# opherlieber/rltime

Measured on AMD Instinct MI355X. Metric: sampled transitions/sec (= learner steps/sec x B x T), IQN-LSTM B=512 T=80 84x84x4, higher is better.
Workload: dtype f32

## Files before the change

### include/mirl.h

```cpp
#ifndef MIRL_H
#define MIRL_H

#include <stdint.h>

#ifdef __cplusplus
extern "C" {
#endif

#define MIRL_OK 0
#define MIRL_NEED_MORE 1
#define MIRL_ERR_ARG (-1)
#define MIRL_ERR_HIP (-2)
#define MIRL_ERR_STATE (-3)
#define MIRL_ERR_NOGPU (-4)

#define MIRL_MODE_UNIFORM 0
#define MIRL_MODE_PER 1

typedef struct mirl_replay mirl_replay;

typedef struct mirl_replay_config {
  int64_t size;
  int32_t num_envs;
  int32_t env_base;
// ... 128 lines not shown
                  double row_scale, float* row_loss, float* dq, float* td, void* stream);
int mirl_loss_iqn(int64_t M, int32_t N, int32_t Nt, int32_t A, const float* z,
                  const float* taus, const int64_t* actions, const float* targets,
                  const float* weights, double kappa, double row_scale,
                  float* row_loss, float* dz, float* abs_td, void* stream);

int mirl_q_target_c51(int64_t M, int32_t A, int32_t Z, const float* logits_target, const float* logits_select,
                      const float* support, const float* returns, const float* nsteps, const float* masks,
                      double gamma, double vmin, double vmax, double delta_z, int32_t projection,
                      float* targets, void* stream);
int mirl_loss_c51(int64_t M, int32_t A, int32_t Z, const float* logits, const int64_t* actions,
                  const float* targets, const float* weights, int32_t mode, double kappa, double row_scale,
                  float* row_loss, float* dlogits, float* report, void* stream);

int mirl_lstm_cell_fwd(int32_t B, int32_t H, float* gates, const float* c_in, const float* keep_next,
                       float* h_out, float* c_out, float* h_next, float* c_next, void* stream);
int mirl_lstm_seq_supported(int32_t T, int32_t B, int32_t H);
int mirl_lstm_seq_workspace_bytes(int32_t B, int32_t H, int64_t* bytes);
int mirl_lstm_seq_fwd(int32_t T, int32_t B, int32_t H, float* gx, const float* w_hh, const float* h0,
                      const float* c0, const float* keep, float* out, float* c_all, float* hm, float* cm,
                      float* h_last, float* c_last, int32_t save_gates, void* workspace, void* stream);
int mirl_lstm_seq_status(int32_t* status);
int mirl_lstm_seq_fwd_grid(int32_t B, int32_t H, int32_t* workgroups, int64_t* lds_bytes, int32_t* compute_units,
                           int32_t* per_compute_unit);
int mirl_lstm_seq_bwd_supported(int32_t T, int32_t B, int32_t H);
int mirl_lstm_seq_bwd_workspace_bytes(int32_t B, int32_t H, int64_t* bytes);
int mirl_lstm_seq_bwd(int32_t T, int32_t B, int32_t H, float* gates, const float* w_hh, const float* c_all,
                      const float* cm, const float* d_out, const float* keep, void* workspace, void* stream);
int mirl_lstm_cell_bwd(int32_t B, int32_t H, float* gates, const float* c_t, const float* c_in,
                       const float* d_out, const float* dh_rec, float* dc_rec, const float* keep_next,
                       int32_t first, void* stream);

int mirl_frames_to_f32_nhwc(int64_t N, int32_t C, int32_t HW, const uint8_t* src, float scale,
                            float* dst, void* stream);
int mirl_frames_to_f32_nhwc_ex(int64_t N, int32_t C, int32_t HW, const uint8_t* src, float scale,
                               float* dst, int32_t per_wg, int32_t flags, void* stream);

int mirl_conv1_u8_supported(int32_t C, int32_t H, int32_t W, int32_t F, int32_t K, int32_t S);
int mirl_conv1_u8_wpk_floats(int64_t* out);
int mirl_conv1_bf16_set(int32_t mode);
int mirl_conv1_wrw_bf16_set(int32_t mode);
int mirl_conv1_u8_fwd(int64_t N, int32_t H, int32_t W, const uint8_t* x, const float* weight,
                      int64_t ws_o, int64_t ws_c, int64_t ws_h, int64_t ws_w, const float* bias,
                      float scale, float* wpk, float* y, void* stream);
int mirl_conv1_u8_fwd_ex(int64_t N, int32_t H, int32_t W, const uint8_t* x, const float* weight,
                         int64_t ws_o, int64_t ws_c, int64_t ws_h, int64_t ws_w, const float* bias,
                         float scale, float* wpk, float* y, int32_t flags, void* stream);

int mirl_conv1_u8_wrw_scratch_floats(int64_t* out);
int mirl_conv1_u8_wrw(int64_t N, int32_t H, int32_t W, const uint8_t* x, const float* g, float scale,
                      float* scratch, float* dw, int64_t ws_o, int64_t ws_c, int64_t ws_h, int64_t ws_w,
                      void* stream);
int mirl_conv1_u8_wrw_ex(int64_t N, int32_t H, int32_t W, const uint8_t* x, const float* g, float scale,
                         float* scratch, float* dw, int64_t ws_o, int64_t ws_c, int64_t ws_h, int64_t ws_w,
                         int32_t flags, void* stream);
int mirl_conv1_u8_wrw_masked(int64_t N, int32_t H, int32_t W, const uint8_t* x, const float* dy, const float* y, float scale,
                             float* scratch, float* dw, int64_t ws_o, int64_t ws_c, int64_t ws_h, int64_t ws_w,
                             float* db, void* stream);

int mirl_conv2_bwd_data_supported(int32_t C, int32_t F, int32_t K, int32_t S, int32_t IH, int32_t IW,
                                  int32_t OH, int32_t OW);
int mirl_conv2_bwd_data(int64_t N, int32_t OH, int32_t OW, const float* g, const float* weight,
                        int64_t ws_o, int64_t ws_c, int64_t ws_h, int64_t ws_w, float* wpk, float* dx,
                        void* stream);
int mirl_conv2_bwd_data_wpk_floats(int64_t* floats);
int mirl_conv2_bwd_data_ex(int64_t N, int32_t OH, int32_t OW, const float* g, const float* weight, int64_t ws_o,
                           int64_t ws_c, int64_t ws_h, int64_t ws_w, float* wpk, int64_t wpk_floats, float* dx, int32_t pipe,
                           void* stream);
int mirl_conv3_bwd_data_supported(int32_t C, int32_t F, int32_t K, int32_t S, int32_t IH, int32_t IW, int32_t OH, int32_t OW);
int mirl_conv3_bwd_data_wpk_floats(int64_t* floats);
int mirl_conv3_bwd_data(int64_t N, int32_t OH, int32_t OW, const float* g, const float* weight, int64_t ws_o,
                        int64_t ws_c, int64_t ws_h, int64_t ws_w, float* wpk, int64_t wpk_floats, float* dx, void* stream);

int mirl_gemm3_supported(int32_t layout, int64_t M, int64_t N, int64_t K);
int mirl_gemm3_workspace_bytes(int32_t layout, int64_t M, int64_t N, int64_t K, int64_t* bytes);
int mirl_gemm3(int32_t layout, int64_t M, int64_t N, int64_t K, const float* A, int64_t lda,
               const float* B, int64_t ldb, float* C, int64_t ldc, const float* bias, int32_t relu,
               void* workspace, int64_t workspace_bytes, void* stream);
int mirl_gemm3_mid_set(int32_t mode);
int mirl_gemm3_nt_mul(int64_t M, int64_t N, int64_t K, const float* A, int64_t lda, const float* B,
                      int64_t ldb, float* C, int64_t ldc, const float* bias, int32_t relu,
                      const float* mul, int64_t ldmul, int32_t group_shift, float* pre, int64_t ldpre,
                      void* stream);
int mirl_gemm3_head_workspace_bytes(int64_t M, int64_t N, int64_t* bytes);
int mirl_gemm3_nt_head(int64_t M, int64_t N, int64_t K, const float* A, int64_t lda, const float* B, int64_t ldb,
                       float* C, int64_t ldc, const float* bias, int32_t relu, const float* w2, int32_t O,
                       const float* bias2, float* out2, int64_t ldo, void* workspace, int64_t workspace_bytes, void* stream);
int mirl_gemm3_nn_qp_partial_rows(int64_t M, int64_t* rows);
int mirl_gemm3_nn_qp(int64_t M, int64_t N, int64_t K, const float* A, int64_t lda, const float* B, int64_t ldb,
                     const float* emb, int64_t ldemb, const float* x, int64_t ldx, float* d_pre, int64_t ldd,
                     float* dx, int64_t lddx, float* db_partial, void* stream);

int mirl_conv3_fwd_supported(int32_t C, int32_t F, int32_t KH, int32_t KW, int32_t S, int32_t H, int32_t W);
int mirl_conv3_fwd(int64_t N, int32_t H, int32_t W, int32_t C, int32_t F, int32_t KH, int32_t KW, int32_t S,
                   const float* x, const float* w, const float* bias, int32_t relu, float* y, void* stream);

int mirl_conv_wrw_b3_supported(int32_t C, int32_t F, int32_t KH, int32_t KW, int32_t S, int32_t H, int32_t W);
int mirl_conv_wrw_b3_scratch_bytes(int32_t C, int32_t F, int32_t KH, int32_t KW, int64_t* bytes);
int mirl_conv_wrw_b3(int64_t N, int32_t H, int32_t W, int32_t C, int32_t F, int32_t KH, int32_t KW, int32_t S,
                     const float* x, const float* g, void* scratch, int64_t scratch_bytes, float* dw, void* stream);

int mirl_bias_relu_rows(int64_t rows, int32_t C, float* y, const float* bias, void* stream);
int mirl_colsum_blocks(int64_t rows, int32_t C, int32_t* blocks);
int mirl_relu_bwd_bias_rows(int64_t rows, int32_t C, const float* dy, const float* y, float* g,
                            float* db, float* partial, int32_t blocks, void* stream);
int mirl_cos_embed(int64_t rows, int32_t D, const float* tau, const float* freq, float* phi, void* stream);
int mirl_cos_embed_rng(int64_t rows, int32_t D, uint64_t seed, const uint64_t* step, const float* freq,
                       float* phi, float* tau_out, void* stream);
int mirl_iqn_mul_fwd(int64_t M, int32_t N, int32_t C, const float* x, const float* emb, float* out, void* stream);
int mirl_iqn_mul_bwd(int64_t M, int32_t N, int32_t C, const float* g, const float* emb, const float* x,
                     float* d_pre, float* dx, float* db, float* partial, int32_t blocks, void* stream);

int mirl_dueling_tail_bwd(int64_t M, int32_t H1, int32_t Hv, int32_t A, int32_t Q, const float* ga,
                          const float* gv, const float* wo, const float* wq, const float* both,
                          float* g, float* db, float* partial, int32_t blocks, void* stream);
int mirl_dueling_tail_bwd_w(int64_t M, int32_t H1, int32_t Hv, int32_t A, int32_t Q, const float* ga,
                            const float* gv, const float* wo, const float* wq, const float* both, float* g,
                            float* db, float* partial, int32_t blocks, float* dwj, float* partial_w,
                            void* stream);

int mirl_actor_head(int32_t E, int32_t N, int32_t A, const float* adv, const float* val, int32_t Q,
                    const double* eps, const double* expo, double eps_min, const float* u, const int64_t* rnd,
                    int32_t* actions, float* qvalues, float* eps_used, void* stream);
int mirl_actor_head_rng(int32_t E, int32_t N, int32_t A, const float* adv, int32_t adv_pitch, const float* val, int32_t Q,
                        const double* eps, const double* expo, double eps_min, uint64_t rng_seed,
                        const uint64_t* rng_step, int32_t* actions, float* qvalues, float* eps_used, void* stream);
int mirl_actor_head_c51(int32_t E, int32_t A, int32_t Z, const float* adv, int32_t adv_pitch, const float* val,
                        int32_t val_pitch, const float* support, const double* eps, const double* expo, double eps_min,
                        const float* u, const int64_t* rnd, uint64_t rng_seed, const uint64_t* rng_step,
                        int32_t* actions, float* qvalues, float* eps_used, void* stream);
int mirl_stack_shift(int32_t E, int32_t P, int32_t plane_bytes, const uint8_t* in, uint8_t* out,
                     const uint8_t* newest, const uint8_t* dones, void* stream);
#define MIRL_STEP_ADVANCE (~0ull)
int mirl_actor_pre(int32_t E, int32_t H, int32_t A, const float* rewards_raw, const uint8_t* dones,
                   const int32_t* actions, const float* h, const float* c, float* xh_tail, int64_t xh_pitch,
                   float* c_in, float* state_pack, float* initials, float* rewards_out, uint8_t* dones_out,
                   int32_t clip_rewards, float* ep_reward, int32_t* ep_len, float* out_reward, int32_t* out_len,
                   int32_t* action_counts, uint64_t* rng_step, uint64_t step, void* stream);
int mirl_synth_env_step(int32_t E, int64_t frame_bytes, const uint8_t* pool, int32_t pool_n, uint64_t* clock, int32_t slot,
                        uint64_t seed, float p_neg, float p_nonpos, float p_done, uint8_t* obs, float* rewards,
                        uint8_t* dones, void* stream);
int mirl_act_conv_supported(int32_t layer, int32_t Ci, int32_t Co, int32_t k, int32_t stride, int32_t Hi, int32_t Wi);
int mirl_act_conv_fwd(int32_t layer, int64_t frames, int32_t Hi, int32_t Wi, const float* x, const float* w_taps,
                      const float* bias, float* y, int64_t y_frame_pitch, void* stream);
int mirl_act_lstm_supported(int32_t E, int32_t H, int32_t K);
int mirl_act_lstm_workspace_bytes(int32_t E, int32_t H, int32_t K, int64_t* bytes);
int mirl_act_lstm_fwd(int32_t E, int32_t H, int32_t K, const float* xh, int64_t xh_pitch, const float* w, const float* bias,
                      const float* c_in, float* h_out, float* c_out, void* workspace, void* stream);
int mirl_act_embed(int32_t E, int32_t N, int32_t H, int32_t D, const float* h, const float* freq, const float* taus,
                   uint64_t seed, const uint64_t* step, const float* wq, const float* bq, float* x, float* tau_out, void* stream);
int mirl_act_head_supported(int32_t E, int32_t N, int32_t H, int32_t D, int32_t HID, int32_t NO);
int mirl_act_head_parts(int32_t HID, int32_t NO, int32_t* parts, int32_t* pitch);
int mirl_act_head_hidden(int32_t R, int32_t H, int32_t HID, int32_t NO, const float* x, const float* wfc, const float* bfc,
                         const float* wout, float* part, void* stream);
int mirl_act_head_select(int32_t E, int32_t N, int32_t A, int32_t parts, int32_t pitch, const float* part, const float* bout,
                         int32_t has_val, const double* eps, const double* expo, double eps_min, uint64_t rng_seed,
                         const uint64_t* rng_step, int32_t* actions, float* qvalues, void* stream);
int mirl_synth_env_step_pre(int32_t E, int64_t frame_bytes, const uint8_t* pool, int32_t pool_n, uint64_t* clock, int32_t slot,
                            uint64_t seed, float p_neg, float p_nonpos, float p_done, uint8_t* obs, float* rewards,
                            uint8_t* dones, int32_t H, int32_t A, const int32_t* actions, const float* h, const float* c,
                            float* xh_tail, int64_t xh_pitch, float* c_in, float* state_pack, float* initials,
                            float* rewards_out, uint8_t* dones_out, int32_t clip_rewards, float* ep_reward, int32_t* ep_len,
                            float* out_reward, int32_t* out_len, int32_t* action_counts, uint64_t* rng_step, uint64_t step,
                            void* stream);
int mirl_catch_env_step(int32_t E, int32_t P, int32_t S, int32_t G, int32_t V, int32_t A, const int32_t* actions, void* state,
                        uint64_t* clock, int32_t slot, uint64_t seed, int32_t reset_all, uint8_t* obs, float* rewards,
// ... 62 lines not shown
```

### rltime_amd/_lib.py

```python
import ctypes as C
import os

import torch

_HERE = os.path.dirname(os.path.abspath(__file__))
LIB_PATH = os.path.join(_HERE, "librltime_hip.so")

MIRL_OK = 0
MIRL_NEED_MORE = 1
MODE_UNIFORM = 0
MODE_PER = 1
INT32_MIN = -2 ** 31


MIRL_OK, MIRL_ERR_ARG, MIRL_ERR_HIP, MIRL_ERR_STATE, MIRL_ERR_NOGPU = 0, -1, -2, -3, -4


class MirlError(RuntimeError):
    code = None


class ReplayConfig(C.Structure):
    _fields_ = [
        ("size", C.c_int64),
# ... 45 lines not shown


class Batch(C.Structure):
    _fields_ = [
        ("frames", C.c_void_p),
        ("extra", C.c_void_p),
        ("state", C.c_void_p),
        ("initials", C.c_void_p),
        ("returns", C.c_void_p),
        ("nsteps", C.c_void_p),
        ("masks", C.c_void_p),
        ("actions", C.c_void_p),
        ("policy", C.c_void_p),
        ("weights", C.c_void_p),
        ("loss_indices", C.c_void_p),
    ]


def _load():
    if not os.path.isfile(LIB_PATH):
        raise MirlError(
            "%s not found: build it with `python -c 'import __graft_entry__ as g; "
            "g.build()'` (rltime_amd/csrc/build.sh). rltime_amd has no CPU "
            "fallback." % LIB_PATH)
    lib = C.CDLL(LIB_PATH)
    lib.mirl_last_error.restype = C.c_char_p
    return lib


lib = _load()

_vp, _i32, _i64, _u64, _f64 = C.c_void_p, C.c_int32, C.c_int64, C.c_uint64, C.c_double
_P = C.POINTER

_SIGNATURES = {
    "mirl_device_count": [],
    "mirl_replay_create": [_P(ReplayConfig), _P(_vp)],
    "mirl_replay_destroy": [_vp],
    "mirl_replay_ingest": [_vp, _P(Ingest), _vp],
    "mirl_replay_ingest_plan": [_vp, _i32, _i32, _vp, _vp],
    "mirl_replay_ingest_planned": [_vp, _i32, _P(Ingest), _vp],
    "mirl_ingest_fused_set": [_i32],
    "mirl_replay_prime_stack": [_vp, _vp, _i64, _vp],
    "mirl_replay_needed_feed_count": [_vp, _i32, _i32, _P(_i64)],
    "mirl_replay_sample": [_vp, _i32, _f64, _vp, _u64, _vp, _vp, _vp, _vp, _vp, _vp, _vp],
    "mirl_replay_sample_ready": [_vp, _i32, _P(_i32)],
    "mirl_replay_sample_skip": [_vp, _i32],
    "mirl_replay_tree_root": [_vp, _vp, _vp],
    "mirl_replay_sample_global": [_vp, _i32, _i32, _i32, _i32, _i32, _vp, _f64, _u64, _vp, _vp, _vp, _vp, _vp, _vp, _vp, _vp],
    "mirl_replay_profile": [_vp, _i32, _P(_i64), _P(_f64)],
    "mirl_profile_set": [_i32],
    "mirl_profile_collect": [_P(_i32)],
    "mirl_profile_get": [_i32, C.c_char_p, _i32, _P(_i64), _P(_f64), _P(_f64)],
    "mirl_profile_get_flop": [_i32, _vp],
    "mirl_profile_reset": [],
    "mirl_replay_save": [_vp, C.c_char_p],
    "mirl_replay_load": [_vp, C.c_char_p],
    "mirl_replay_uniform_total": [_vp, _P(_i64)],
    "mirl_replay_set_train_quota": [_vp, _i64],
    "mirl_replay_state_rows": [_vp, _P(_i32), _P(_i32)],
    "mirl_replay_gather": [_vp, _i32, _vp, _vp, _vp, _vp, _P(Batch), _vp],
    "mirl_replay_update_losses": [_vp, _i64, _vp, _vp, _vp],
    "mirl_replay_stats": [_vp, _P(_i64), _P(_i64), _P(_i64), _P(_i64), _P(_i64)],
    "mirl_replay_env_meta": [_vp, _vp, _vp],
    "mirl_replay_free_slots": [_vp, _vp, _P(_i64)],
    "mirl_replay_slot_table": [_vp, _vp, _vp],
    "mirl_replay_tree_nodes": [_vp, _vp, _vp, _vp],
    "mirl_replay_tree_set_leaves": [_vp, _i64, _vp, _vp, _vp],
    "mirl_replay_tree_find": [_vp, _i32, _vp, _vp, _vp],
    "mirl_replay_losses_peek": [_vp, _i32, _i64, _i32, _vp],
    "mirl_q_target_dqn": [_i64, _i32, _vp, _vp, _vp, _vp, _vp, _f64, _f64, _vp, _vp],
    "mirl_q_target_iqn": [_i64, _i32, _i32, _i32, _vp, _vp, _vp, _vp, _vp, _f64, _f64, _vp, _vp],
    "mirl_loss_dqn": [_i64, _i32, _vp, _vp, _vp, _vp, _f64, _i32, _f64, _vp, _vp, _vp, _vp],
    "mirl_loss_iqn": [_i64, _i32, _i32, _i32, _vp, _vp, _vp, _vp, _vp, _f64, _f64, _vp, _vp, _vp, _vp],
    "mirl_q_target_c51": [_i64, _i32, _i32, _vp, _vp, _vp, _vp, _vp, _vp, _f64, _f64, _f64, _f64, _i32, _vp, _vp],
    "mirl_loss_c51": [_i64, _i32, _i32, _vp, _vp, _vp, _vp, _i32, _f64, _f64, _vp, _vp, _vp, _vp],
    "mirl_actor_head_c51": [_i32, _i32, _i32, _vp, _i32, _vp, _i32, _vp, _vp, _vp, _f64, _vp, _vp, _u64, _vp, _vp, _vp, _vp, _vp],
    "mirl_lstm_cell_fwd": [_i32, _i32, _vp, _vp, _vp, _vp, _vp, _vp, _vp, _vp],
    "mirl_lstm_seq_supported": [_i32, _i32, _i32],
    "mirl_lstm_seq_workspace_bytes": [_i32, _i32, _P(_i64)],
    "mirl_lstm_seq_fwd": [_i32, _i32, _i32, _vp, _vp, _vp, _vp, _vp, _vp, _vp, _vp, _vp, _vp, _vp, _i32, _vp, _vp],
    "mirl_lstm_seq_status": [_P(_i32)],
    "mirl_gemm3_mid_set": [_i32],
    "mirl_lstm_seq_fwd_grid": [_i32, _i32, _P(_i32), _P(_i64), _P(_i32), _P(_i32)],
    "mirl_lstm_seq_bwd_supported": [_i32, _i32, _i32],
    "mirl_lstm_seq_bwd_workspace_bytes": [_i32, _i32, _P(_i64)],
    "mirl_lstm_seq_bwd": [_i32, _i32, _i32, _vp, _vp, _vp, _vp, _vp, _vp, _vp, _vp],
    "mirl_lstm_cell_bwd": [_i32, _i32, _vp, _vp, _vp, _vp, _vp, _vp, _vp, _i32, _vp],
    "mirl_frames_to_f32_nhwc": [_i64, _i32, _i32, _vp, C.c_float, _vp, _vp],
    "mirl_frames_to_f32_nhwc_ex": [_i64, _i32, _i32, _vp, C.c_float, _vp, _i32, _i32, _vp],
    "mirl_conv1_u8_supported": [_i32, _i32, _i32, _i32, _i32, _i32],
    "mirl_conv1_bf16_set": [_i32],
    "mirl_conv1_wrw_bf16_set": [_i32],
    "mirl_conv1_u8_wpk_floats": [_P(_i64)],
    "mirl_conv1_u8_fwd": [_i64, _i32, _i32, _vp, _vp, _i64, _i64, _i64, _i64, _vp, C.c_float, _vp, _vp, _vp],
    "mirl_conv1_u8_fwd_ex": [_i64, _i32, _i32, _vp, _vp, _i64, _i64, _i64, _i64, _vp, C.c_float, _vp, _vp, _i32, _vp],
    "mirl_conv1_u8_wrw_scratch_floats": [_P(_i64)],
    "mirl_conv1_u8_wrw_ex": [_i64, _i32, _i32, _vp, _vp, C.c_float, _vp, _vp, _i64, _i64, _i64, _i64, _i32, _vp],
    "mirl_conv1_u8_wrw_masked": [_i64, _i32, _i32, _vp, _vp, _vp, C.c_float, _vp, _vp, _i64, _i64, _i64, _i64, _vp, _vp],
    "mirl_conv1_u8_wrw": [_i64, _i32, _i32, _vp, _vp, C.c_float, _vp, _vp, _i64, _i64, _i64, _i64, _vp],
    "mirl_conv2_bwd_data_supported": [_i32, _i32, _i32, _i32, _i32, _i32, _i32, _i32],
    "mirl_conv2_bwd_data": [_i64, _i32, _i32, _vp, _vp, _i64, _i64, _i64, _i64, _vp, _vp, _vp],
    "mirl_conv2_bwd_data_wpk_floats": [_P(_i64)],
    "mirl_conv3_bwd_data_supported": [_i32, _i32, _i32, _i32, _i32, _i32, _i32, _i32],
    "mirl_conv3_bwd_data_wpk_floats": [_P(_i64)],
    "mirl_conv3_bwd_data": [_i64, _i32, _i32, _vp, _vp, _i64, _i64, _i64, _i64, _vp, _i64, _vp, _vp],
    "mirl_conv2_bwd_data_ex": [_i64, _i32, _i32, _vp, _vp, _i64, _i64, _i64, _i64, _vp, _i64, _vp, _i32, _vp],
    "mirl_conv3_fwd_supported": [_i32, _i32, _i32, _i32, _i32, _i32, _i32],
    "mirl_conv3_fwd": [_i64, _i32, _i32, _i32, _i32, _i32, _i32, _i32, _vp, _vp, _vp, _i32, _vp, _vp],
    "mirl_conv_wrw_b3_supported": [_i32, _i32, _i32, _i32, _i32, _i32, _i32],
    "mirl_conv_wrw_b3_scratch_bytes": [_i32, _i32, _i32, _i32, _P(_i64)],
    "mirl_conv_wrw_b3": [_i64, _i32, _i32, _i32, _i32, _i32, _i32, _i32, _vp, _vp, _vp, _i64, _vp, _vp],
    "mirl_gemm3_supported": [_i32, _i64, _i64, _i64],
    "mirl_gemm3_workspace_bytes": [_i32, _i64, _i64, _i64, _P(_i64)],
    "mirl_gemm3": [_i32, _i64, _i64, _i64, _vp, _i64, _vp, _i64, _vp, _i64, _vp, _i32, _vp, _i64, _vp],
    "mirl_gemm3_nt_mul": [_i64, _i64, _i64, _vp, _i64, _vp, _i64, _vp, _i64, _vp, _i32, _vp, _i64, _i32, _vp, _i64, _vp],
    "mirl_gemm3_nn_qp_partial_rows": [_i64, _P(_i64)],
    "mirl_gemm3_nn_qp": [_i64, _i64, _i64, _vp, _i64, _vp, _i64, _vp, _i64, _vp, _i64, _vp, _i64, _vp, _i64, _vp, _vp],
    "mirl_gemm3_head_workspace_bytes": [_i64, _i64, _P(_i64)],
    "mirl_gemm3_nt_head": [_i64, _i64, _i64, _vp, _i64, _vp, _i64, _vp, _i64, _vp, _i32, _vp, _i32, _vp, _vp, _i64, _vp, _i64, _vp],
    "mirl_act_conv_supported": [_i32, _i32, _i32, _i32, _i32, _i32, _i32],
    "mirl_act_conv_fwd": [_i32, _i64, _i32, _i32, _vp, _vp, _vp, _vp, _i64, _vp],
    "mirl_act_lstm_supported": [_i32, _i32, _i32],
    "mirl_act_lstm_workspace_bytes": [_i32, _i32, _i32, _P(_i64)],
    "mirl_act_lstm_fwd": [_i32, _i32, _i32, _vp, _i64, _vp, _vp, _vp, _vp, _vp, _vp, _vp],
    "mirl_act_embed": [_i32, _i32, _i32, _i32, _vp, _vp, _vp, _u64, _vp, _vp, _vp, _vp, _vp, _vp],
    "mirl_act_head_supported": [_i32, _i32, _i32, _i32, _i32, _i32],
    "mirl_act_head_parts": [_i32, _i32, _P(_i32), _P(_i32)],
    "mirl_act_head_hidden": [_i32, _i32, _i32, _i32, _vp, _vp, _vp, _vp, _vp, _vp],
    "mirl_act_head_select": [_i32, _i32, _i32, _i32, _i32, _vp, _vp, _i32, _vp, _vp, _f64, _u64, _vp, _vp, _vp, _vp],
    "mirl_bias_relu_rows": [_i64, _i32, _vp, _vp, _vp],
    "mirl_colsum_blocks": [_i64, _i32, _P(_i32)],
    "mirl_relu_bwd_bias_rows": [_i64, _i32, _vp, _vp, _vp, _vp, _vp, _i32, _vp],
    "mirl_cos_embed": [_i64, _i32, _vp, _vp, _vp, _vp],
    "mirl_cos_embed_rng": [_i64, _i32, _u64, _vp, _vp, _vp, _vp, _vp],
    "mirl_adam_clip_workspace_bytes": [_i32, _vp, _vp],
    "mirl_adam_clip_step": [_i32, _vp, _vp, _vp, _vp, _vp, _vp, _f64, _vp, _f64, _f64, _f64, _f64, _vp, _i64, _vp, _vp],
    "mirl_adam_clip_step_guarded": [_i32, _vp, _vp, _vp, _vp, _vp, _vp, _f64, _vp, _f64, _f64, _f64, _f64, _vp, _i64, _vp, _vp, _vp],
    "mirl_step_guard_open": [_vp, _vp, _i64, _vp, _i32, _vp],
    "mirl_replay_update_losses_guarded": [_vp, _i64, _vp, _vp, _vp, _vp],
    "mirl_lstm_seq_status_device": [_P(_vp)],
    "mirl_iqn_mul_fwd": [_i64, _i32, _i32, _vp, _vp, _vp, _vp],
    "mirl_iqn_mul_bwd": [_i64, _i32, _i32, _vp, _vp, _vp, _vp, _vp, _vp, _vp, _i32, _vp],
    "mirl_dueling_tail_bwd": [_i64, _i32, _i32, _i32, _i32, _vp, _vp, _vp, _vp, _vp, _vp, _vp, _vp, _i32, _vp],
    "mirl_dueling_tail_bwd_w": [_i64, _i32, _i32, _i32, _i32, _vp, _vp, _vp, _vp, _vp, _vp, _vp, _vp, _i32, _vp, _vp, _vp],
    "mirl_actor_head": [_i32, _i32, _i32, _vp, _vp, _i32, _vp, _vp, _f64, _vp, _vp, _vp, _vp, _vp, _vp],
    "mirl_actor_head_rng": [_i32, _i32, _i32, _vp, _i32, _vp, _i32, _vp, _vp, _f64, _u64, _vp, _vp, _vp, _vp, _vp],
    "mirl_stack_shift": [_i32, _i32, _i32, _vp, _vp, _vp, _vp, _vp],
    "mirl_synth_env_step": [_i32, _i64, _vp, _i32, _vp, _i32, _u64, C.c_float, C.c_float, C.c_float, _vp, _vp, _vp, _vp],
    "mirl_synth_env_step_pre": [_i32, _i64, _vp, _i32, _vp, _i32, _u64, C.c_float, C.c_float, C.c_float, _vp, _vp, _vp,
                                _i32, _i32, _vp, _vp, _vp, _vp, _i64, _vp, _vp, _vp, _vp, _vp, _i32, _vp, _vp, _vp, _vp, _vp, _vp, _u64, _vp],
    "mirl_catch_env_step": [_i32, _i32, _i32, _i32, _i32, _i32, _vp, _vp, _vp, _i32, _u64, _i32, _vp, _vp, _vp, _vp],
    "mirl_catch_env_step_pre": [_i32, _i32, _i32, _i32, _i32, _i32, _vp, _vp, _vp, _i32, _u64, _i32, _vp, _vp, _vp,
                                _i32, _i32, _vp, _vp, _vp, _vp, _i64, _vp, _vp, _vp, _vp, _vp, _i32, _vp, _vp, _vp, _vp, _vp, _vp, _u64, _vp],
    "mirl_actor_pre": [_i32, _i32, _i32, _vp, _vp, _vp, _vp, _vp, _vp, _i64, _vp, _vp, _vp, _vp, _vp, _i32, _vp, _vp, _vp, _vp,
                       _vp, _vp, _u64, _vp],
    "mirl_episode_track": [_i32, _i32, _vp, _vp, _vp, _vp, _vp, _vp, _vp, _vp, _vp],
    "mirl_eval_count": [_i32, _i32, _i32, _vp, _vp, _vp, _vp, _vp, _vp, _vp, _vp, _vp],
    "mirl_copy_bytes": [_vp, _vp, _i64, _vp],
    "mirl_copy_bytes_ex": [_vp, _vp, _i64, _i32, _vp],
    "mirl_book_create": [_P(ReplayConfig), _P(_vp)],
    "mirl_book_destroy": [_vp],
    "mirl_book_ingest": [_vp, _i32, _vp],
    "mirl_book_stats": [_vp, _P(_i64), _P(_i64), _P(_i64), _P(_i64), _P(_i64)],
    "mirl_book_env_meta": [_vp, _vp, _vp],
    "mirl_book_free_slots": [_vp, _vp, _P(_i64)],
# ... 65 lines not shown
```

### rltime_amd/csrc/gemm3.hip

```cpp
#include "common.hpp"
#include "split3.hpp"
#include <stdlib.h>

namespace mirl {

struct G3Args {
  const float* A; const float* B; float* C; const float* bias;
  int64_t M, N, K;
  int64_t lda, ldb, ldc;
  int relu;
  int mt, nt;
  int splits;
  int steps_per_split;
  const float* mul; int64_t ldmul; int mul_shift;
  float* pre; int64_t ldpre;
  int vec_ok;
  const float* w2; float* part;
  float* gsum; int64_t ldgsum;
};


template <bool KC>
struct G3Loader {
  const float* p[2];
  int64_t step;
  int64_t ld;
  int lds_off;
  __device__ __forceinline__ void init(const float* base, int64_t ld_, int64_t row0, int64_t rows, int64_t k0, int t) {
    ld = ld_;
    if (KC) {
      const int r = t >> 2, kq = t & 3;
#pragma unroll
      for (int h = 0; h < 2; ++h) {
        int64_t row = row0 + r + 128 * h; if (row > rows - 1) row = rows - 1;
        p[h] = base + row * ld + k0 + kq * 4;
      }
      step = 16;
      lds_off = r * G3_PITCH + kq * 8;
    } else {
      const int kq = t >> 7, r = t & 127;
#pragma unroll
      for (int h = 0; h < 2; ++h) {
        int64_t row = row0 + r + 128 * h; if (row > rows - 1) row = rows - 1;
        p[h] = base + (k0 + kq * 4) * ld + row;
      }
      step = 16 * ld;
      lds_off = r * G3_PITCH + kq * 8;
    }
  }
  __device__ __forceinline__ void load(float (&v)[2][4]) {
#pragma unroll
    for (int h = 0; h < 2; ++h) {
      if (KC) {
        const float4 q = *reinterpret_cast<const float4*>(p[h]);
        v[h][0] = q.x; v[h][1] = q.y; v[h][2] = q.z; v[h][3] = q.w;
      } else {
#pragma unroll
        for (int e = 0; e < 4; ++e) v[h][e] = p[h][e * ld];
      }
      p[h] += step;
    }
  }
  __device__ __forceinline__ void store(char* planes, const float (&v)[2][4]) const {
#pragma unroll
    for (int h = 0; h < 2; ++h) {
      uint2 a, b, c;
      g3_split4(v[h], a, b, c);
      char* d = planes + lds_off + h * 128 * G3_PITCH;
      *reinterpret_cast<uint2*>(d) = a;
      *reinterpret_cast<uint2*>(d + G3_PLANE) = b;
      *reinterpret_cast<uint2*>(d + 2 * G3_PLANE) = c;
    }
  }
};

template <int TI>
__device__ __forceinline__ void g3_compute(const char* stage, g3_f32x16 (&acc)[TI][2], int a_off, int b_off) {
  const char* pa = stage + a_off;
  const char* pb = stage + 3 * G3_PLANE + b_off;
  constexpr int PA[6] = {2, 0, 1, 1, 0, 0};
  constexpr int PB[6] = {0, 2, 1, 0, 1, 0};
  g3_bf16x8 b[3][2];
#pragma unroll
  for (int p = 0; p < 3; ++p)
#pragma unroll
// ... 331 lines not shown
  auto store_b = [&](char* planes) {
    uint2 h, m, lo;
    g3_split4(vb, h, m, lo);
    *reinterpret_cast<uint2*>(planes + b_lds) = h;
    *reinterpret_cast<uint2*>(planes + G3M_BPLANE + b_lds) = m;
    *reinterpret_cast<uint2*>(planes + 2 * G3M_BPLANE + b_lds) = lo;
  };
  const int a_off = (wm * 128 + (lane & 31)) * G3_PITCH + (lane >> 5) * 16;
  const int b_off = (wn * 32 + (lane & 31)) * G3_PITCH + (lane >> 5) * 16;
  const bool stage_first = (wu >> 2) & 1;

  g3_f32x16 acc[4];
#pragma unroll
  for (int i = 0; i < 4; ++i)
#pragma unroll
    for (int r = 0; r < 16; ++r) acc[i][r] = 0.0f;
  constexpr int PA[6] = {2, 0, 1, 1, 0, 0};
  constexpr int PB[6] = {0, 2, 1, 0, 1, 0};

  if (nk > 0) { la.load(va); load_b(); la.store(g3_lds, va); store_b(g3_lds + 3 * G3_PLANE); }
  if (nk > 1) { la.load(va); load_b(); }
  g3_barrier();
  for (int64_t k = 0; k < nk; ++k) {
    const char* cur = g3_lds + (k & 1) * G3M_STAGE;
    char* nxt = g3_lds + ((k + 1) & 1) * G3M_STAGE;
    if (stage_first) {
      if (k + 1 < nk) { la.store(nxt, va); store_b(nxt + 3 * G3_PLANE); }
      if (k + 2 < nk) { la.load(va); load_b(); }
    }
    {
      const char* pa = cur + a_off;
      const char* pbf = cur + 3 * G3_PLANE + b_off;
      g3_bf16x8 bf[3];
#pragma unroll
      for (int p = 0; p < 3; ++p) bf[p] = *reinterpret_cast<const g3_bf16x8*>(pbf + p * G3M_BPLANE);
      __builtin_amdgcn_s_setprio(1);
#pragma unroll
      for (int ih = 0; ih < 2; ++ih) {
        g3_bf16x8 a[3][2];
#pragma unroll
        for (int p = 0; p < 3; ++p)
#pragma unroll
          for (int i = 0; i < 2; ++i) a[p][i] = *reinterpret_cast<const g3_bf16x8*>(pa + p * G3_PLANE + (ih * 2 + i) * 32 * G3_PITCH);
#pragma unroll
        for (int c = 0; c < 6; ++c)
#pragma unroll
          for (int i = 0; i < 2; ++i) acc[ih * 2 + i] = g3_mfma(a[PA[c]][i], bf[PB[c]], acc[ih * 2 + i]);
      }
      __builtin_amdgcn_s_setprio(0);
    }
    if (!stage_first) {
      if (k + 1 < nk) { la.store(nxt, va); store_b(nxt + 3 * G3_PLANE); }
      if (k + 2 < nk) { la.load(va); load_b(); }
    }
    g3_barrier();
  }

  float* tl = reinterpret_cast<float*>(g3_lds) + wu * (32 * G3M_EPITCH);
  const int c4 = lane & 7;
  const int64_t col = n0 + wn * 32 + c4 * 4;
  float4 bv = make_float4(0.f, 0.f, 0.f, 0.f);
  if (g.bias && col < g.N) bv = *reinterpret_cast<const float4*>(g.bias + col);
#pragma unroll
  for (int i = 0; i < 4; ++i) {
#pragma unroll
    for (int r = 0; r < 16; ++r)
      tl[((r & 3) + 8 * (r >> 2) + 4 * (lane >> 5)) * G3M_EPITCH + (lane & 31)] = acc[i][r];
    asm volatile("s_waitcnt lgkmcnt(0)" ::: "memory");
#pragma unroll
    for (int q = 0; q < 4; ++q) {
      const int rl = q * 8 + (lane >> 3);
      const int64_t row = m0 + wm * 128 + i * 32 + rl;
      float4 v = *reinterpret_cast<const float4*>(tl + rl * G3M_EPITCH + c4 * 4);
      if (row < g.M && col < g.N) {
        v.x += bv.x; v.y += bv.y; v.z += bv.z; v.w += bv.w;
        if (g.relu) { v.x = v.x > 0.f ? v.x : 0.f; v.y = v.y > 0.f ? v.y : 0.f; v.z = v.z > 0.f ? v.z : 0.f; v.w = v.w > 0.f ? v.w : 0.f; }
        *reinterpret_cast<float4*>(g.C + row * g.ldc + col) = v;
      }
    }
    asm volatile("s_waitcnt lgkmcnt(0)" ::: "memory");
  }
}

__global__ void __launch_bounds__(256)
k_gemm3_reduce(const float* __restrict__ partial, int splits, int64_t M, int64_t N, float* __restrict__ out, int64_t ldc) {
  const int64_t n4 = N >> 2;
  const int64_t total = M * n4;
  for (int64_t i = (int64_t)blockIdx.x * blockDim.x + threadIdx.x; i < total; i += (int64_t)gridDim.x * blockDim.x) {
    const int64_t row = i / n4, c4 = i - row * n4;
    float4 s = make_float4(0.f, 0.f, 0.f, 0.f);
    for (int k = 0; k < splits; ++k) {
      const float4 v = *reinterpret_cast<const float4*>(partial + ((int64_t)k * M + row) * N + c4 * 4);
      s.x += v.x; s.y += v.y; s.z += v.z; s.w += v.w;
    }
    *reinterpret_cast<float4*>(out + row * ldc + c4 * 4) = s;
  }
}

__global__ void __launch_bounds__(256)
k_g3_head_reduce(const float* __restrict__ part, int ncb, int64_t M, int O, const float* __restrict__ bias2,
                 float* __restrict__ out, int64_t ldo) {
  for (int64_t i = (int64_t)blockIdx.x * 256 + threadIdx.x; i < M * 2; i += (int64_t)gridDim.x * 256) {
    const int64_t row = i >> 1;
    const int half = (int)(i & 1);
    float4 sum = make_float4(0.f, 0.f, 0.f, 0.f);
    for (int cb = 0; cb < ncb; ++cb) {
      const float4 v = *reinterpret_cast<const float4*>(part + ((int64_t)cb * M + row) * 8 + half * 4);
      sum.x += v.x; sum.y += v.y; sum.z += v.z; sum.w += v.w;
    }
    const float r[4] = {sum.x, sum.y, sum.z, sum.w};
#pragma unroll
    for (int e = 0; e < 4; ++e) {
      const int o = half * 4 + e;
      if (o < O) out[row * ldo + o] = r[e] + (bias2 ? bias2[o] : 0.f);
    }
  }
}

static int g_g3_mid_mode = -1;

static int g3_splits(int64_t M, int64_t N, int64_t K) {
  const int64_t tiles = ((M + 255) / 256) * ((N + 255) / 256);
  int64_t s = 8 * ((256 + 8 * tiles - 1) / (8 * tiles));
  const int64_t nk = K / 16;
  while (s > 8 && nk / s < 64) s -= 8;
  return (int)s;
}

}

extern "C" int mirl_gemm3_supported(int32_t layout, int64_t M, int64_t N, int64_t K) {
  if (layout < 0 || layout > 2) return 0;
  if (M < 1 || N < 1 || K < 16 || (K % 16)) return 0;
  if (M >= (1LL << 31) || N >= (1LL << 31)) return 0;
  if (layout == 2) {
    if (N % 4) return 0;
    if (K / 16 < 8) return 0;
  }
  return 1;
}

extern "C" int mirl_gemm3_workspace_bytes(int32_t layout, int64_t M, int64_t N, int64_t K, int64_t* bytes) {
  using namespace mirl;
  if (!bytes) return fail(MIRL_ERR_ARG, "gemm3_workspace_bytes: null out");
  if (!mirl_gemm3_supported(layout, M, N, K)) return fail(MIRL_ERR_ARG, "gemm3: unsupported layout / shape");
  *bytes = layout == 2 ? (int64_t)g3_splits(M, N, K) * M * N * (int64_t)sizeof(float) : 0;
  return MIRL_OK;
}

namespace mirl {
struct G3Opt {
  const float* mul = nullptr; int64_t ldmul = 0; int32_t mul_shift = 0;
  float* pre = nullptr; int64_t ldpre = 0;
  const float* w2 = nullptr; float* part = nullptr;
  float* gsum = nullptr; int64_t ldgsum = 0;
};

struct G3Kernel { const void* fn; const char* name; };
static G3Kernel g3_kernel(int layout, int vec, bool mul, bool w2, bool gsum, bool narrow) {
  static const void* const plain[4][2] = {{(const void*)k_gemm3<true, true, 0, false>, (const void*)k_gemm3<true, true, 0, true>},
                                          {(const void*)k_gemm3<true, false, 0, false>, (const void*)k_gemm3<true, false, 0, true>},
                                          {nullptr , (const void*)k_gemm3<false, false, 0, true>},
                                          {(const void*)k_gemm3<true, true, 1, false>, (const void*)k_gemm3<true, true, 1, true>}};
  static const char* const names[4] = {"k_gemm3_nt", "k_gemm3_nn", "k_gemm3_tn", "k_gemm3_nt_mul"};
  if (gsum) return {(const void*)k_gemm3<true, false, 3, true>, "k_gemm3_nn_qp"};
  if (w2) return {(const void*)k_gemm3<true, true, 2, true>, "k_gemm3_nt_head"};
  if (narrow) return {(const void*)k_gemm3<false, false, 0, true, true>, "k_gemm3_tn"};
  const int which = mul ? 3 : layout;
  return {plain[which][vec], names[which]};
}
}

static int g3_launch(int32_t layout, int64_t M, int64_t N, int64_t K, const float* A, int64_t lda, const float* B,
                     int64_t ldb, float* C, int64_t ldc, const float* bias, int32_t relu, void* workspace,
                     int64_t workspace_bytes, void* stream, const mirl::G3Opt& o = mirl::G3Opt()) {
  using namespace mirl;
  if (!mirl_gemm3_supported(layout, M, N, K)) return fail(MIRL_ERR_ARG, "gemm3: unsupported layout / shape");
  if (!A || !B || (!C && !o.w2)) return fail(MIRL_ERR_ARG, "gemm3: null operand");
  const bool akc = layout != 2, bkc = layout == 0;
  if (akc && ((lda % 4) || !aligned16(A) || lda < K)) return fail(MIRL_ERR_ARG, "gemm3: A must be 16-byte aligned with lda % 4 == 0");
  if (bkc && ((ldb % 4) || !aligned16(B) || ldb < K)) return fail(MIRL_ERR_ARG, "gemm3: B must be 16-byte aligned with ldb % 4 == 0");
  if (!akc && lda < M) return fail(MIRL_ERR_ARG, "gemm3: lda < M");
  if (!bkc && ldb < N) return fail(MIRL_ERR_ARG, "gemm3: ldb < N");
  if (ldc < N) return fail(MIRL_ERR_ARG, "gemm3: ldc < N");
  if (layout == 2 && (bias || relu)) return fail(MIRL_ERR_ARG, "gemm3: no epilogue with split K");
  hipStream_t st = (hipStream_t)stream;
  G3Args g;
  g.A = A; g.B = B; g.C = C; g.bias = bias; g.M = M; g.N = N; g.K = K; g.lda = lda; g.ldb = ldb; g.ldc = ldc;
  g.relu = relu ? 1 : 0;
  g.mul = o.mul; g.ldmul = o.ldmul; g.mul_shift = o.mul_shift; g.pre = o.pre; g.ldpre = o.ldpre;
  g.w2 = o.w2; g.part = o.part; g.gsum = o.gsum; g.ldgsum = o.ldgsum;
  g.vec_ok = (N % 4 == 0) && (ldc % 4 == 0) && aligned16(C, o.w2, bias, o.mul, o.pre) && (!o.mul || o.ldmul % 4 == 0) && (!o.pre || o.ldpre % 4 == 0);
  g.mt = (int)((M + 255) / 256); g.nt = (int)((N + 255) / 256);
  g.splits = 1; g.steps_per_split = (int)(K / 16);
  unsigned grid = (unsigned)(8 * ((g.mt + 7) / 8) * g.nt);
  if (K <= 128) {
    const unsigned resident = (unsigned)(cu_count() / 8 * 8);
    if (resident && grid > resident) grid = resident;
  }
  if (layout == 2) {
    g.splits = g3_splits(M, N, K);
    const int64_t need = (int64_t)g.splits * M * N * (int64_t)sizeof(float);
    if (!workspace || workspace_bytes < need || (ldc % 4) || !aligned16(workspace, C))
      return fail(MIRL_ERR_ARG, "gemm3: split-K workspace too small / misaligned");
    g.steps_per_split = (int)((K / 16 + g.splits - 1) / g.splits);
    g.C = (float*)workspace; g.ldc = N;
    grid = (unsigned)(g.mt * g.nt * g.splits);
  }
  const int vec = g.vec_ok ? 1 : 0;
  const double flop = 2.0 * (double)M * (double)N * (double)K;
  if (g_g3_mid_mode != 0 && layout == 0 && !o.mul && !o.w2 && !o.gsum && vec && (N % 4) == 0 && (int64_t)g.mt * g.nt < 192 && N > 128 &&
      ((int64_t)g.mt * ((N + G3M_BROWS - 1) / G3M_BROWS) >= 192 || (int64_t)g.mt * g.nt < 24)) {
    if (int rc = raise_lds_limit(k_gemm3_mid, G3M_LDS)) return rc;
    g.nt = (int)((N + G3M_BROWS - 1) / G3M_BROWS);
    const unsigned mgrid = (unsigned)(8 * ((g.mt + 7) / 8) * g.nt);
    ProfScope ps("k_gemm3_nt_mid", 4.0 * ((double)M * K + (double)N * K + (double)M * N), st, flop);
    void* kargs[] = {(void*)&g};
    MIRL_HIP(hipLaunchKernel((const void*)k_gemm3_mid, dim3(mgrid), dim3(512), kargs, G3M_LDS, st));
    return MIRL_OK;
  }
  if (o.gsum) {
    if (!vec || layout != 1 || !o.mul || o.mul_shift != 5 || !o.pre || !o.part || (o.ldgsum % 4) || !aligned16(o.gsum, o.part) || (M % 32))
      return fail(MIRL_ERR_ARG, "gemm3: the fused feature-product backward needs the NN form, groups of 32 rows and 16-byte aligned rows");
  } else if (o.w2) {
    if (!vec || layout != 0 || o.mul || !o.part) return fail(MIRL_ERR_ARG, "gemm3: the fused following layer needs the NT form with 16-byte aligned rows");
  }
  const G3Kernel k = g3_kernel(layout, vec, o.mul, o.w2, o.gsum, layout == 2 && N <= 64);
  if (int rc = raise_lds_limit(k.fn, G3_LDS)) return rc;
  {
    double bytes = 4.0 * ((double)M * K + (double)N * K + (double)M * N * (layout == 2 ? (double)g.splits : 1.0));
    if (o.mul) bytes += 4.0 * ((o.pre ? (double)M * N : 0.0) + (double)(M >> o.mul_shift) * N * (o.gsum ? 2.0 : 1.0));
    if (o.w2) bytes += 4.0 * (8.0 * (double)N + 8.0 * (double)M * (double)((N + 63) / 64)) - (C ? 0.0 : 4.0 * (double)M * N);
    ProfScope ps(k.name, bytes, st, flop);
    void* kargs[] = {(void*)&g};
    MIRL_HIP(hipLaunchKernel(k.fn, dim3(grid), dim3(512), kargs, G3_LDS, st));
  }
  if (layout == 2) {
    ProfScope ps("k_gemm3_reduce", (double)(g.splits + 1) * (double)M * (double)N * 4.0, st);
    hipLaunchKernelGGL(k_gemm3_reduce, dim3(capped_grid((M * (N / 4) + 255) / 256, 4096)), dim3(256), 0, st, (const float*)workspace, g.splits, M, N, C, ldc);
    MIRL_LAUNCH_CHECK();
  }
  return MIRL_OK;
}

extern "C" int mirl_gemm3(int32_t layout, int64_t M, int64_t N, int64_t K, const float* A, int64_t lda, const float* B,
                          int64_t ldb, float* C, int64_t ldc, const float* bias, int32_t relu, void* workspace,
                          int64_t workspace_bytes, void* stream) {
  return g3_launch(layout, M, N, K, A, lda, B, ldb, C, ldc, bias, relu, workspace, workspace_bytes, stream);
}

extern "C" int mirl_gemm3_mid_set(int32_t mode) {
  if (mode < -1 || mode > 1) return mirl::fail(MIRL_ERR_ARG, "gemm3_mid_set: mode is -1 (default), 0 or 1");
  mirl::g_g3_mid_mode = mode;
  return MIRL_OK;
}

extern "C" int mirl_gemm3_nt_mul(int64_t M, int64_t N, int64_t K, const float* A, int64_t lda, const float* B, int64_t ldb,
                                 float* C, int64_t ldc, const float* bias, int32_t relu, const float* mul, int64_t ldmul,
                                 int32_t group_shift, float* pre, int64_t ldpre, void* stream) {
  using namespace mirl;
  if (!mul || group_shift < 0 || group_shift > 30 || ldmul < N || (pre && ldpre < N))
    return fail(MIRL_ERR_ARG, "gemm3_nt_mul: bad multiplier / pre-activation arguments");
  G3Opt o;
  o.mul = mul; o.ldmul = ldmul; o.mul_shift = group_shift; o.pre = pre; o.ldpre = ldpre;
  return g3_launch(0, M, N, K, A, lda, B, ldb, C, ldc, bias, relu, nullptr, 0, stream, o);
}

extern "C" int mirl_gemm3_nn_qp_partial_rows(int64_t M, int64_t* rows) {
  if (!rows || M < 1) return mirl::fail(MIRL_ERR_ARG, "gemm3_nn_qp_partial_rows: M >= 1");
  *rows = 2 * ((M + 255) / 256);
  return MIRL_OK;
}

extern "C" int mirl_gemm3_nn_qp(int64_t M, int64_t N, int64_t K, const float* A, int64_t lda, const float* B, int64_t ldb,
                                const float* emb, int64_t ldemb, const float* x, int64_t ldx, float* d_pre, int64_t ldd,
                                float* dx, int64_t lddx, float* db_partial, void* stream) {
  using namespace mirl;
  if (!emb || !x || !d_pre || !dx || !db_partial || ldemb < N || ldx < N || lddx < N || (ldemb % 4) || !aligned16(emb))
    return fail(MIRL_ERR_ARG, "gemm3_nn_qp: bad embedding / feature / output arguments");
  G3Opt o;
  o.mul = x; o.ldmul = ldx; o.mul_shift = 5; o.pre = const_cast<float*>(emb); o.ldpre = ldemb;
  o.part = db_partial; o.gsum = dx; o.ldgsum = lddx;
  return g3_launch(1, M, N, K, A, lda, B, ldb, d_pre, ldd, nullptr, 0, nullptr, 0, stream, o);
}

extern "C" int mirl_gemm3_head_workspace_bytes(int64_t M, int64_t N, int64_t* bytes) {
  if (!bytes || M < 1 || N < 1) return mirl::fail(MIRL_ERR_ARG, "bad gemm3_head_workspace_bytes arguments");
  *bytes = 8 * (int64_t)sizeof(float) * M * ((N + 255) / 256 * 4);
  return MIRL_OK;
}

extern "C" int mirl_gemm3_nt_head(int64_t M, int64_t N, int64_t K, const float* A, int64_t lda, const float* B, int64_t ldb,
                                  float* C, int64_t ldc, const float* bias, int32_t relu, const float* w2, int32_t O,
                                  const float* bias2, float* out2, int64_t ldo, void* workspace, int64_t workspace_bytes,
                                  void* stream) {
  using namespace mirl;
  int64_t need = 0;
  if (O < 1 || O > 8 || !w2 || !out2 || ldo < O || !workspace || mirl_gemm3_head_workspace_bytes(M, N, &need) || workspace_bytes < need ||
      !aligned16(workspace) || (N % 4))
    return fail(MIRL_ERR_ARG, "bad gemm3_nt_head arguments (1 <= O <= 8, N % 4 == 0, 16-byte aligned workspace of head_workspace_bytes)");
  if (!C) ldc = N;
  G3Opt o;
  o.w2 = w2; o.part = (float*)workspace;
  if (int rc = g3_launch(0, M, N, K, A, lda, B, ldb, C, ldc, bias, relu, nullptr, 0, stream, o)) return rc;
  const int ncb = (int)((N + 255) / 256 * 4);
  hipStream_t st = (hipStream_t)stream;
  ProfScope ps("k_g3_head_reduce", 4.0 * (8.0 * ncb + O) * (double)M, st);
  hipLaunchKernelGGL(k_g3_head_reduce, dim3(capped_grid((2 * M + 255) / 256, 16384)), dim3(256), 0, st, (const float*)workspace, ncb, M, (int)O, bias2, out2, ldo);
  MIRL_LAUNCH_CHECK();
  return MIRL_OK;
}
```

Measured before the change: 481,500.

## Add register-resident B GEMM kernel for small-K fused multiply NT form

Adds a specialized kernel for the NT GEMM with per-group multiplier (IQN quantile embedding product) when K<=64. It splits B into three bf16 parts once per block and keeps them in registers, then loops persistently over 32-row M tiles, prefetching the next A tile while running the MFMAs. The multiplier row is hoisted when groups span 32 rows. The goal is to avoid LDS staging and repeated B loads for this thin-K shape, at the cost of more register pressure and a fixed 2-blocks-per-CU persistent grid.

```diff
diff --git a/include/mirl.h b/include/mirl.h
--- a/include/mirl.h
+++ b/include/mirl.h
@@ -234,6 +234,9 @@
                       int64_t ldb, float* C, int64_t ldc, const float* bias, int32_t relu,
                       const float* mul, int64_t ldmul, int32_t group_shift, float* pre, int64_t ldpre,
                       void* stream);
+int mirl_gemm3_mul_form_set(int32_t mode);
+int mirl_gemm3_mul_form_supported(int64_t M, int64_t N, int64_t K);
+int mirl_gemm3_mul_form_last(void);
 int mirl_gemm3_head_workspace_bytes(int64_t M, int64_t N, int64_t* bytes);
 int mirl_gemm3_nt_head(int64_t M, int64_t N, int64_t K, const float* A, int64_t lda, const float* B, int64_t ldb,
                        float* C, int64_t ldc, const float* bias, int32_t relu, const float* w2, int32_t O,
diff --git a/rltime_amd/_lib.py b/rltime_amd/_lib.py
--- a/rltime_amd/_lib.py
+++ b/rltime_amd/_lib.py
@@ -151,6 +151,9 @@
     "mirl_lstm_seq_fwd": [_i32, _i32, _i32, _vp, _vp, _vp, _vp, _vp, _vp, _vp, _vp, _vp, _vp, _vp, _i32, _vp, _vp],
     "mirl_lstm_seq_status": [_P(_i32)],
     "mirl_gemm3_mid_set": [_i32],
+    "mirl_gemm3_mul_form_set": [_i32],
+    "mirl_gemm3_mul_form_supported": [_i64, _i64, _i64],
+    "mirl_gemm3_mul_form_last": [],
     "mirl_lstm_seq_fwd_grid": [_i32, _i32, _P(_i32), _P(_i64), _P(_i32), _P(_i32)],
     "mirl_lstm_seq_bwd_supported": [_i32, _i32, _i32],
     "mirl_lstm_seq_bwd_workspace_bytes": [_i32, _i32, _P(_i64)],
diff --git a/rltime_amd/csrc/gemm3.hip b/rltime_amd/csrc/gemm3.hip
--- a/rltime_amd/csrc/gemm3.hip
+++ b/rltime_amd/csrc/gemm3.hip
@@ -1,6 +1,7 @@
 #include "common.hpp"
 #include "split3.hpp"
 #include <stdlib.h>
+#include <atomic>
 
 namespace mirl {
 
@@ -498,6 +499,130 @@
   }
 }
 
+__device__ __forceinline__ void qr_split8(const float4& q0, const float4& q1, g3_bf16x8& h, g3_bf16x8& m, g3_bf16x8& lo) {
+  const float x0[4] = {q0.x, q0.y, q0.z, q0.w}, x1[4] = {q1.x, q1.y, q1.z, q1.w};
+  uint2 h0, m0, l0, h1, m1, l1;
+  g3_split4(x0, h0, m0, l0);
+  g3_split4(x1, h1, m1, l1);
+  h = __builtin_bit_cast(g3_bf16x8, make_uint4(h0.x, h0.y, h1.x, h1.y));
+  m = __builtin_bit_cast(g3_bf16x8, make_uint4(m0.x, m0.y, m1.x, m1.y));
+  lo = __builtin_bit_cast(g3_bf16x8, make_uint4(l0.x, l0.y, l1.x, l1.y));
+}
+
+template <bool PRE, bool HOIST>
+__device__ __forceinline__ void qr_store(const G3Args& g, const float* tl, int64_t m0, int64_t col, int lane, const float4& bv, const float4& mg) {
+  const int c4 = lane & 15;
+  const int last = g.M - m0 < 32 ? (int)(g.M - m0) - 1 : 31;
+  float4 v[8], m[8];
+#pragma unroll
+  for (int q = 0; q < 8; ++q) {
+    int rl = q * 4 + (lane >> 4); if (rl > last) rl = last;
+    v[q] = *reinterpret_cast<const float4*>(tl + rl * G3_EPITCH + c4 * 4);
+    if (HOIST) m[q] = mg;
+    else m[q] = *reinterpret_cast<const float4*>(g.mul + ((m0 + rl) >> g.mul_shift) * g.ldmul + col);
+  }
+#pragma unroll
+  for (int q = 0; q < 8; ++q) { v[q].x += bv.x; v[q].y += bv.y; v[q].z += bv.z; v[q].w += bv.w; }
+  if (g.relu) {
+#pragma unroll
+    for (int q = 0; q < 8; ++q) { v[q].x = v[q].x > 0.f ? v[q].x : 0.f; v[q].y = v[q].y > 0.f ? v[q].y : 0.f; v[q].z = v[q].z > 0.f ? v[q].z : 0.f; v[q].w = v[q].w > 0.f ? v[q].w : 0.f; }
+  }
+#pragma unroll
+  for (int q = 0; q < 8; ++q) {
+    int rl = q * 4 + (lane >> 4); if (rl > last) rl = last;
+    const int64_t row = m0 + rl;
+    float4 w = v[q];
+    if (PRE) __builtin_nontemporal_store(g3_f32x4{w.x, w.y, w.z, w.w}, reinterpret_cast<g3_f32x4*>(g.pre + row * g.ldpre + col));
+    w.x *= m[q].x; w.y *= m[q].y; w.z *= m[q].z; w.w *= m[q].w;
+    __builtin_nontemporal_store(g3_f32x4{w.x, w.y, w.z, w.w}, reinterpret_cast<g3_f32x4*>(g.C + row * g.ldc + col));
+  }
+}
+
+template <int NK, bool PRE, bool HOIST>
+__global__ void __launch_bounds__(256, 2)
+k_gemm3_qreg(G3Args g) {
+  __shared__ __attribute__((aligned(16))) float qr_lds[4][32 * G3_EPITCH];
+  const int lane = threadIdx.x & 63;
+  const int wu = __builtin_amdgcn_readfirstlane(threadIdx.x >> 6);
+  const int b = blockIdx.x, xcd = b & 7, l = b >> 3, L = gridDim.x >> 3;
+  const int jt = l % g.nt;
+  const int64_t n0 = ((int64_t)jt * 4 + wu) * 64;
+  if (n0 >= g.N) return;
+  const int E = ((g.mt + 7) / 8) * g.nt;
+  const int r32 = lane & 31, kg = lane >> 5;
+
+  g3_bf16x8 bp[3][2][NK];
+#pragma unroll
+  for (int j = 0; j < 2; ++j) {
+    const float* pb = g.B + (n0 + j * 32 + r32) * g.ldb + 8 * kg;
+#pragma unroll
+    for (int s = 0; s < NK; ++s)
+      qr_split8(*reinterpret_cast<const float4*>(pb + 16 * s), *reinterpret_cast<const float4*>(pb + 16 * s + 4), bp[0][j][s], bp[1][j][s], bp[2][j][s]);
+  }
+  const int64_t col = n0 + (lane & 15) * 4;
+  float4 bv = make_float4(0.f, 0.f, 0.f, 0.f);
+  if (g.bias) bv = *reinterpret_cast<const float4*>(g.bias + col);
+  float* tl = qr_lds[wu];
+
+  int e = l, it = 0;
+  for (; e < E; e += L) { it = (e / g.nt) * 8 + xcd; if (it < g.mt) break; }
+  if (e >= E) return;
+
+  float4 raw[NK][2];
+  float4 mgn = make_float4(0.f, 0.f, 0.f, 0.f);
+  auto request = [&](int tile) {
+    int64_t row = (int64_t)tile * 32 + r32; if (row > g.M - 1) row = g.M - 1;
+    const float* pa = g.A + row * g.lda + 8 * kg;
+#pragma unroll
+    for (int s = 0; s < NK; ++s) {
+      raw[s][0] = *reinterpret_cast<const float4*>(pa + 16 * s);
+      raw[s][1] = *reinterpret_cast<const float4*>(pa + 16 * s + 4);
+    }
+    if (HOIST) mgn = *reinterpret_cast<const float4*>(g.mul + (((int64_t)tile * 32) >> g.mul_shift) * g.ldmul + col);
+  };
+  request(it);
+  __builtin_amdgcn_s_waitcnt(0x0F70);
+
+  constexpr int PA[6] = {2, 0, 1, 1, 0, 0};
+  constexpr int PB[6] = {0, 2, 1, 0, 1, 0};
+  while (true) {
+    const int64_t m0 = (int64_t)it * 32;
+    g3_bf16x8 ap[3][NK];
+#pragma unroll
+    for (int s = 0; s < NK; ++s) qr_split8(raw[s][0], raw[s][1], ap[0][s], ap[1][s], ap[2][s]);
+    const float4 mg = mgn;
+
+    const int it_now = it;
+    for (e += L; e < E; e += L) { it = (e / g.nt) * 8 + xcd; if (it < g.mt) break; }
+    const bool more = e < E;
+    request(more ? it : it_now);
+
+    g3_f32x16 acc[2];
+#pragma unroll
+    for (int j = 0; j < 2; ++j)
+#pragma unroll
+      for (int r = 0; r < 16; ++r) acc[j][r] = 0.0f;
+    __builtin_amdgcn_s_setprio(1);
+#pragma unroll
+    for (int s = 0; s < NK; ++s)
+#pragma unroll
+      for (int c = 0; c < 6; ++c)
+#pragma unroll
+        for (int j = 0; j < 2; ++j) acc[j] = g3_mfma(ap[PA[c]][s], bp[PB[c]][j][s], acc[j]);
+    __builtin_amdgcn_s_setprio(0);
+
+#pragma unroll
+    for (int j = 0; j < 2; ++j)
+#pragma unroll
+      for (int r = 0; r < 16; ++r)
+        tl[((r & 3) + 8 * (r >> 2) + 4 * (lane >> 5)) * G3_EPITCH + j * 32 + r32] = acc[j][r];
+    asm volatile("s_waitcnt lgkmcnt(0)" ::: "memory");
+    qr_store<PRE, HOIST>(g, tl, m0, col, lane, bv, mg);
+    asm volatile("s_waitcnt lgkmcnt(0)" ::: "memory");
+    if (!more) break;
+  }
+}
+
 __global__ void __launch_bounds__(256)
 k_gemm3_reduce(const float* __restrict__ partial, int splits, int64_t M, int64_t N, float* __restrict__ out, int64_t ldc) {
   const int64_t n4 = N >> 2;
@@ -534,6 +659,13 @@
 }
 
 static int g_g3_mid_mode = -1;
+static std::atomic<int> g_g3_mul_form{-1};
+static std::atomic<int> g_g3_mul_form_last{-1};
+
+static bool g3_qreg_shape(int64_t M, int64_t N, int64_t K) {
+  if (M < 1 || M >= (1LL << 31) || N < 64 || N >= (1LL << 31) || (N % 64) || (K % 16) || K < 16 || K > 64) return false;
+  return ((M + 31) / 32 + 7) / 8 * ((N + 255) / 256) < (1LL << 30);
+}
 
 static int g3_splits(int64_t M, int64_t N, int64_t K) {
   const int64_t tiles = ((M + 255) / 256) * ((N + 255) / 256);
@@ -635,6 +767,25 @@
     MIRL_HIP(hipLaunchKernel((const void*)k_gemm3_mid, dim3(mgrid), dim3(512), kargs, G3M_LDS, st));
     return MIRL_OK;
   }
+  if (layout == 0 && o.mul && !o.w2 && !o.gsum) {
+    const bool qreg = g_g3_mul_form.load() != 0 && vec && g3_qreg_shape(M, N, K);
+    g_g3_mul_form_last.store(qreg ? 1 : 0);
+    if (qreg) {
+#define MIRL_QREG(NK) {{(const void*)k_gemm3_qreg<NK, false, false>, (const void*)k_gemm3_qreg<NK, false, true>}, {(const void*)k_gemm3_qreg<NK, true, false>, (const void*)k_gemm3_qreg<NK, true, true>}}
+      static const void* const fns[4][2][2] = {MIRL_QREG(1), MIRL_QREG(2), MIRL_QREG(3), MIRL_QREG(4)};
+#undef MIRL_QREG
+      g.mt = (int)((M + 31) / 32); g.nt = (int)((N + 255) / 256);
+      const int64_t E = (int64_t)((g.mt + 7) / 8) * g.nt;
+      int64_t L = (int64_t)(2 * cu_count() / 8) / g.nt * g.nt;
+      if (L < g.nt) L = g.nt;
+      if (L > E) L = E;
+      const double bytes = 4.0 * ((double)M * K + (double)N * K + (double)M * N + (o.pre ? (double)M * N : 0.0) + (double)(M >> o.mul_shift) * N);
+      ProfScope ps("k_gemm3_nt_mul", bytes, st, flop);
+      void* kargs[] = {(void*)&g};
+      MIRL_HIP(hipLaunchKernel(fns[K / 16 - 1][o.pre ? 1 : 0][o.mul_shift >= 5 ? 1 : 0], dim3((unsigned)(8 * L)), dim3(256), kargs, 0, st));
+      return MIRL_OK;
+    }
+  }
   if (o.gsum) {
     if (!vec || layout != 1 || !o.mul || o.mul_shift != 5 || !o.pre || !o.part || (o.ldgsum % 4) || !aligned16(o.gsum, o.part) || (M % 32))
       return fail(MIRL_ERR_ARG, "gemm3: the fused feature-product backward needs the NN form, groups of 32 rows and 16-byte aligned rows");
@@ -670,6 +821,16 @@
   mirl::g_g3_mid_mode = mode;
   return MIRL_OK;
 }
+
+extern "C" int mirl_gemm3_mul_form_set(int32_t mode) {
+  if (mode < -1 || mode > 1) return mirl::fail(MIRL_ERR_ARG, "gemm3_mul_form_set: mode is -1 (automatic), 0 or 1");
+  mirl::g_g3_mul_form.store(mode);
+  return MIRL_OK;
+}
+
+extern "C" int mirl_gemm3_mul_form_supported(int64_t M, int64_t N, int64_t K) { return mirl::g3_qreg_shape(M, N, K) ? 1 : 0; }
+
+extern "C" int mirl_gemm3_mul_form_last(void) { return mirl::g_g3_mul_form_last.load(); }
 
 extern "C" int mirl_gemm3_nt_mul(int64_t M, int64_t N, int64_t K, const float* A, int64_t lda, const float* B, int64_t ldb,
                                  float* C, int64_t ldc, const float* bias, int32_t relu, const float* mul, int64_t ldmul,
```

After: 482,800 (median of 5 runs). Within noise of the previous version (+0.3%).
